# bnbowman/pbccs

Measured on AMD Instinct MI355X. Metric: CCS ZMWs/sec (and GCUPS) at 1/2/4/8 MI355X vs host-CPU ccs, higher is better.
Workload: dtype f64

## Files before the change

### pbccs_amd/csrc/engine.hip

```cpp
#include "engine.hpp"
#include "diploid_kernels.hpp"
#include "refine_repeats.hpp"

#include <hipcub/hipcub.hpp>

#include <algorithm>
#include <mutex>
#include <climits>
#include <cmath>
#include <cstdio>
#include <cstdlib>
#include <cstring>
#include <numeric>
#include <set>
#include <stdexcept>
#include <chrono>
#include <unordered_set>

namespace pbccs {

#define PBCCS_HIP(x)                                                         \
    do {                                                                     \
        hipError_t e_ = (x);                                                 \
        if (e_ != hipSuccess) throw DeviceError(hipGetErrorString(e_));      \
// ... 892 lines not shown
    b.prNot = 1.0 - kMismatchProbability;
    b.prThird = kMismatchProbability / 3.0;
    b.sdn = zmws_.empty() ? std::exp(12.5) : std::exp(zmws_[0].opt.scoreDiff);
    b.stats = profiling_ ? dStats_.ptr : nullptr;
    return b;
}

void ArrowBatch::FillReads(const std::vector<int>& readsIn)
{
    const StreamScope bound(stream_);
    constexpr int kPaths = 4;
    for (int r : readsIn) EnsureCapacity(r);
    auto promote = [&](int r, int p) {
        HRead& h = reads_[r];
        int q = p + 1;
        if (q == 2 && (long long)h.seq.size() + 1 > 4LL * kCoopTallRows) q = 3;
        h.fillPath = q;
        if (q >= 2 && q < kPaths) {
            const long long I = (long long)h.seq.size(), J = h.te - h.ts;
            const bool ck = ckptAll_ > 0 || (ckptK_ > 0 && J >= ckptMinLen_);
            const long long K = ck ? std::max(ckptAll_, ckptK_) : 1;
            const long long want = (I + 1) * (J + 1) / kTallFirstDiv / K + (ck ? 2 * (kCkptTail + 1) * (I + 1) : 0) + 64;
            if (want > h.valCap) {
                h.valCap = want;
                h.valA = valTop_;
                h.valB = valTop_ + h.valCap;
                valTop_ += 2 * h.valCap;
                descDirty_ = true;
            }
        }
        return q;
    };
    Relayout(readsIn);
    std::vector<int> todo[kPaths], serial, done;
    for (int r : readsIn) {
        const int p = reads_[r].fillPath;
        if (p >= kPaths) serial.push_back(r);
        else todo[p].push_back(r);
    }
    auto words = [&](int r) {
        return (int)(reads_[r].seq.size() + 7) / 8 + (reads_[r].te - reads_[r].ts + 8) / 8;
    };
    constexpr int tallG = 64;
    static const int tallRows = env_int("PBCCS_TALL_ROWS", kTallRowsPerLane) == 1 ? 1 : 2;
    const long long chunk = (long long)tallG * tallRows;
    const long long tallGroupLds = (long long)kCoopLdsBytes;
    auto full_rows = [&](int maxI) { return ((long long)maxI + chunk) / chunk * chunk; };
    constexpr int narrowG = kNarrowGroupLanes;
    constexpr int narrowRows = 1;
    auto rows_for = [&](int p, int maxI, int w) -> int {
        if (p == 0) return 0;
        if (p == 1)
            return (64 / narrowG) * coop_group_bytes(kCoopNarrowRows, w, 0) <= kCoopLdsBytes
                       ? kCoopNarrowRows : 0;
        const long long room = (tallGroupLds - (long long)coop_group_bytes(0, w, 0)) / 16 / 64 * 64;
        const long long full = full_rows(maxI);
        if (p == 2) {
            const long long want = std::min<long long>(kCoopTallRows, full);
            return room >= want ? (int)want : 0;
        }
        static const long long hybLds = (long long)env_int("PBCCS_HYBRID_LDS_KB", (int)(kCoopLdsBytes >> 10)) << 10;
        static const long long hybRows = env_int("PBCCS_HYBRID_ROWS", kHybridRows);
        const long long hroom = (std::min<long long>(hybLds, 160 << 10) - (long long)coop_group_bytes(0, w, 0)) / 16 / 64 * 64;
        const long long want = std::min(std::min(full, hroom), hybRows);
        return want >= 64 ? (int)want : 0;
    };
    static const bool pathTrace = std::getenv("PBCCS_FILL_PATHS") != nullptr;
    static const bool pathTrace2 = pathTrace && std::getenv("PBCCS_FILL_PATHS")[0] == '2';
    static const bool fillWork = std::getenv("PBCCS_FILL_WORK") != nullptr;
    for (int attempt = 0;; ++attempt) {
        for (int p = 0; p < kPaths; ++p) {
            std::vector<int> keep;
            for (int r : todo[p]) {
                if (rows_for(p, (int)reads_[r].seq.size(), words(r)) > 0) keep.push_back(r);
                else if (p + 1 < kPaths) todo[p + 1].push_back(r);
                else {
                    reads_[r].fillPath = kPaths;
                    serial.push_back(r);
                }
            }
            todo[p].swap(keep);
        }
        if (std::all_of(todo, todo + kPaths, [](const std::vector<int>& v) { return v.empty(); })) break;
        if (attempt > 8) throw DeviceError("band storage keeps overflowing");
        auto quick = [&](int x) { return reads_[x].filled && reads_[x].flips == 0 ? 1 : 0; };
        auto high = [&](int x) {
            const HRead& h = reads_[x];
            return h.filled && std::max(h.usedA, h.usedB) > 16LL * (h.te - h.ts + 1) ? 0 : 1;
        };
        for (int p = 0; p < kPaths; ++p) {
            auto& v = todo[p];
            if (p >= 2) {
                std::stable_sort(v.begin(), v.end(), [&](int x, int y) {
                    return std::max(reads_[x].usedA, reads_[x].usedB) > std::max(reads_[y].usedA, reads_[y].usedB);
                });
// ... 1517 lines not shown
```

### pbccs_amd/csrc/fill_coop.hip

```cpp
#include "arrow_device.hpp"
#include "arrow_kernels.hpp"
#include "coop_chain.hpp"

#include <algorithm>
#include <cstdlib>
#include <stdexcept>

namespace pbccs {
namespace {

using namespace coop;

template <int G>
struct Task {
    Group<G> g;
    int I, J, L, start;
    const unsigned* rdW;
    const unsigned* tpW;
    const double* ctx;
    double* lds0;
    double* lds1;
    double* glob0;
    double* glob1;
    int hcap;
    int rowsCap;
    bool gcol;
    int ckK;
    bool chainExit;
    int slackDiv;
    double prNot, prThird, sdn;
    double sdnInvLow;
    double sdnInvHigh;
    double devScale;
    double sdnInv;
    int r;
    double* pool;
    unsigned long long* bump;
    long long limit;
    long long* gA;
    long long* gB;
    long long* gCap;

    bool split;
    __device__ __forceinline__ int lrow(int k) const { return split ? (k & 1) * (hcap >> 1) + (k >> 1) : k; }
    __device__ __forceinline__ double* cptr(int b, int k) const
    {
        if (!gcol) return lds0 + (b ? hcap : 0) + lrow(k);
        return k < hcap ? lds0 + (b ? hcap : 0) + lrow(k) : glob0 + (b ? glob1 - glob0 : 0) + (k - hcap);
    }
    __device__ __forceinline__ double cget(int b, int k) const { return *cptr(b, k); }
    __device__ __forceinline__ void cset(int b, int k, double v) const { *cptr(b, k) = v; }
    __device__ __forceinline__ int TBase(int idx) const
    {
        return nib(tpW, max(idx, 0));
    }
    __device__ __forceinline__ int TCtx(int idx) const
    {
        return (start + idx + 1 < L) ? ctx_code(TBase(idx), TBase(idx + 1)) : kCtxZero;
    }
    __device__ __forceinline__ int RB(int x) const
    {
        return nib(rdW, x);
    }
};

struct PassOut {
    long long used;
    long long stored;
    double last;
    double sumL;
    bool tall;
    bool changed;
    bool regrow;
    int maxH;
    double dev;
    int unc;
};

struct Work {
    bool on;
    long long steps;
    long long issues;
};
__device__ __forceinline__ void count_issue(Work& W)
{
    if (W.on) {
        const unsigned long long act = __ballot(1);
        if ((int)(threadIdx.x & 63) == __ffsll((long long)act) - 1) W.issues += 1;
    }
}

__device__ __forceinline__ void col_fence(bool gcol)
{
    if (gcol) __builtin_amdgcn_fence(__ATOMIC_ACQ_REL, "workgroup");
}

__device__ __forceinline__ bool thr_ge(double x, double pm, double lo, double hi, bool& amb)
{
    const bool ge = x >= pm * hi;
    const bool lt = x < pm * lo;
    amb = pm != 0.0 && (pm < 0x1p-960 || (!ge && !lt));
    return ge || pm == 0.0;
}

__device__ __forceinline__ double scan_col_dev(double D, int chunks, int rowsPerChunk)
{
    return D + (4.0 * (double)chunks * (double)rowsPerChunk + 40.0 * (double)chunks + 8.0) * kUnitRoundoff;
}
__device__ __forceinline__ bool near_thr(double x, double t, double margin)
{
    const double mx = fmax(x, t);
    return mx > 0.0 && fabs(x - t) <= margin * mx;
}

template <int G>
__device__ __forceinline__ void copy_vals(int lane, double* __restrict__ dst, const double* __restrict__ src, long long n)
{
    long long k = lane;
    for (; k + 3 * G < n; k += 4 * G) {
        const double x0 = src[k], x1 = src[k + G], x2 = src[k + 2 * G], x3 = src[k + 3 * G];
        dst[k] = x0;
        dst[k + G] = x1;
        dst[k + 2 * G] = x2;
        dst[k + 3 * G] = x3;
    }
    for (; k < n; k += G) dst[k] = src[k];
}

template <int G>
__device__ bool regrow_bands(const Task<G>& T, Band& m, Band& o, bool mIsAlpha, long long need, long long keepO)
{
    if (!T.bump) return false;
    const long long full = (long long)(T.I + 1) * (T.J + 1) + 1;
    long long cap = max(need, keepO);
    cap = max(min(cap + cap / T.slackDiv + 64, full), max(need, keepO));
    unsigned long long base = 0;
    if (T.g.lane == 0) base = atomicAdd(T.bump, (unsigned long long)(2 * cap));
    base = (unsigned long long)__shfl((long long)base, 0, G);
    if (base + 2 * (unsigned long long)cap > (unsigned long long)T.limit) return false;
    __threadfence();
    double* na = T.pool + base;
    double* nb = na + cap;
    double* nm = mIsAlpha ? na : nb;
    double* no = mIsAlpha ? nb : na;
    copy_vals<G>(T.g.lane, no, o.val, keepO);
// ... 21 lines not shown
#pragma unroll
            for (int q = 0; q < 8; ++q) v[q] = m.L(k + q);
#pragma unroll
            for (int q = 0; q < 8; ++q) s = s + v[q];
        }
        for (; k <= J; ++k) s = s + m.L(k);
    }
    return T.g.bcast(s, 0);
}

#ifndef PBCCS_TALL_PREFETCH
#define PBCCS_TALL_PREFETCH 1
#endif
template <int G, int R, bool SCAN, bool GC>
__device__ PassOut coop_alpha(const Task<G>& T, Band& a, Band& o, bool guided, bool selfValid, bool& ovf, long long keepO,
                              Work& W)
{
    constexpr int CH = G * R;
    constexpr bool PF = GC || (G == 64 && PBCCS_TALL_PREFETCH && !SCAN);
    constexpr bool PFS = GC || (G == 64 && PBCCS_TALL_PREFETCH);
    const Band* guide = guided ? &o : nullptr;
    const int I = T.I, J = T.J, lane = T.g.lane;
    PassOut out{0, 0, 0.0, 0.0, false, !selfValid, false, 1, 0.0, 0};
    bool counting = false;
    (void)keepO;
    if (a.cap < 1) ovf = true;
    if (lane == 0) {
        if (!ovf) a.V(0) = 1.0;
        a.R(0) = make_int2(0, 1);
        a.O(0) = 0;
        a.L(0) = 0.0;
    }
    int prev = 0, cur = 1;
    if (lane == 0) T.cset(prev, 0, 1.0);
    int pb = 0, pe = 1;
    double D = 0.0;
    int unc = 0;
    long long used = 1, stored = 1;
    int hb = 1, he = 1;
    int prevCtx = kCtxZero;
    int curBase = T.TBase(0), curCtx = T.TCtx(0);
    int tA = T.TBase(1), tB = T.TBase(2);
    double myF = 1.0;
    int2 gR = make_int2(0, 0), sR = make_int2(0, 0), gN = make_int2(0, 0), sN = make_int2(0, 0);
    {
        const int jj = G == 64 ? 1 + lane : 1;
        if (guide && jj < J) gN = guide->R(jj);
        if (selfValid && jj < J) sN = a.R(jj);
    }
    for (int j = 1; j < J; ++j) {
        const int jb = (j - 1) & (G - 1);
        int gx = 0, gy = 0, sx = 0, sy = 0;
        if constexpr (G == 64) {
            if (jb == 0) {
                gR = gN;
                sR = sN;
                const int jj = j + G + lane;
                if (guide && jj < J) gN = guide->R(jj);
                if (selfValid && jj < J) sN = a.R(jj);
            }
            if (guide) { gx = T.g.bcast(gR.x, jb); gy = T.g.bcast(gR.y, jb); }
            if (selfValid) { sx = T.g.bcast(sR.x, jb); sy = T.g.bcast(sR.y, jb); }
        } else {
            gR = gN;
            sR = sN;
            if (guide && j + 1 < J) gN = guide->R(j + 1);
            if (selfValid && j + 1 < J) sN = a.R(j + 1);
            gx = gR.x; gy = gR.y; sx = sR.x; sy = sR.y;
        }
        (void)jb;
        if (guide) {
            if (gx < gy) { hb = min(gx, hb); he = max(gy, he); }
        }
        if (selfValid) {
            if (sx < sy) { hb = min(sx, hb); he = max(sy, he); }
        }
        const int reqEnd = min(I, he);
        const int nextBase = tA, nextCtx = (T.start + j + 1 < T.L) ? ctx_code(tA, tB) : kCtxZero;
        const int tC = T.TBase(j + 2);
        const double* cp = T.ctx + curCtx * kCtxStride;
        const double* pp = T.ctx + prevCtx * kCtxStride;
        const double pMatch = pp[kM], pDel = pp[kD];
        const double cBranch = cp[kB], cStick3 = cp[kS3];
        const int b = hb;
        double mx = 0.0, aLast[R];
        int e = b, nc = 0;
        if (b < I) {
            double carry = 0.0;
            auto load_prev = [&](int ibx, double (&dst)[R + 1]) {
#pragma unroll
                for (int q = 0; q <= R; ++q) {
                    const int row = ibx - 1 + q;
                    dst[q] = (row >= pb && row < pe) ? T.cget(prev, row - pb) : 0.0;
                }
            };
            double pvN[R + 1];
            if constexpr (PF) load_prev(b + lane * R, pvN);
            for (int i0 = b;; i0 += CH) {
                if ((nc + 1) * CH > T.rowsCap) {
                    out.tall = true;
                    out.used = used;
                    W.steps += nc;
                    return out;
                }
                count_issue(W);
                const int ib = i0 + lane * R;
                double m[R], k[R], d[R], x[R];
                {
                    double pv[R + 1];
                    if constexpr (PF) {
#pragma unroll
                        for (int q = 0; q <= R; ++q) pv[q] = pvN[q];
                        load_prev(ib + CH, pvN);
                    } else {
                        load_prev(ib, pv);
                    }
#pragma unroll
                    for (int r = 0; r < R; ++r) {
                        const int i = ib + r;
                        const int rb = (i >= 1 && i <= I) ? T.RB(i - 1) : 15;
                        const double mpe = pv[r] * (rb == curBase ? T.prNot : T.prThird);
                        m[r] = (i == 1 && j == 1) ? mpe : ((i != 1 && j != 1) ? mpe * pMatch : 0.0);
                        k[r] = (i > 1) ? (rb == nextBase ? cBranch : cStick3) : 0.0;
                        d[r] = (j > 1) ? pv[r + 1] * pDel : 0.0;
                        x[r] = 0.0;
                    }
                }
                bool nz = false;
#pragma unroll
                for (int r = 0; r < R; ++r) nz = nz || m[r] != 0.0 || d[r] != 0.0;
                const unsigned long long nzb = T.g.bits(nz);
                if (carry != 0.0 || nzb != 0) {
                    const int startLane = ((G == 64 || R > 1) && carry == 0.0) ? __ffsll((long long)nzb) - 1 : 0;
                    if constexpr (R == 1) {
                        const int i = ib;
                        if (G == 64 && T.chainExit) {
                            auto maybe_stop = [&](double xv) {
                                const double pmv = fmax(mx, prefix_max<G>(xv));
                                return T.g.bits((i + 1 >= I) || (xv < pmv * T.sdnInvLow && i + 1 >= reqEnd));
                            };
                            x[0] = insertion_chain64_exit(m[0], k[0], d[0], carry, min(reqEnd, I) - 1 - i0, maybe_stop,
                                                          startLane);
                        } else {
                            x[0] = insertion_chain<G>(m[0], k[0], d[0], carry);
                        }
                    } else {
                        auto maybe_stop = [&](const double (&xv)[R]) {
                            double lp = xv[0];
#pragma unroll
                            for (int r = 1; r < R; ++r) lp = fmax(lp, xv[r]);
                            const double ex = shift_up<G>(prefix_max<G>(lp), 0.0);
                            double run = fmax(mx, ex);
                            bool st = false;
#pragma unroll
                            for (int r = 0; r < R; ++r) {
                                run = fmax(run, xv[r]);
                                const int i = ib + r;
                                st = st || (i + 1 >= I) || (xv[r] < run * T.sdnInvLow && i + 1 >= reqEnd);
                            }
                            return T.g.bits(st);
                        };
                        const int firstRow = min(reqEnd, I) - 1 - i0;
                        if constexpr (SCAN) {
                            scan_chain64<R>(m, k, d, carry, x);
                        } else {
                            insertion_chain_rows<G, R>(m, k, d, carry, x, firstRow < 0 ? 0 : firstRow / R, T.chainExit,
                                                       startLane, maybe_stop);
                        }
                    }
                }
                double pmR[R];
                if constexpr (R == 1) {
                    pmR[0] = fmax(mx, prefix_max<G>(x[0]));
                } else {
                    double lp = x[0];
#pragma unroll
                    for (int r = 1; r < R; ++r) lp = fmax(lp, x[r]);
                    double run = fmax(mx, shift_up<G>(prefix_max<G>(lp), 0.0));
#pragma unroll
                    for (int r = 0; r < R; ++r) {
                        run = fmax(run, x[r]);
                        pmR[r] = run;
                    }
                }
                bool ge[R], amb = false;
#pragma unroll
                for (int r = 0; r < R; ++r) {
                    const int i = ib + r;
                    bool a;
                    ge[r] = thr_ge(x[r], pmR[r], T.sdnInvLow, T.sdnInvHigh, a);
                    amb = amb || (a && i + 1 < I && i + 1 >= reqEnd);
                }
                if (__ballot(amb) != 0) {
#pragma unroll
                    for (int r = 0; r < R; ++r) ge[r] = x[r] >= pmR[r] / T.sdn;
                }
                int fs = R;
#pragma unroll
                for (int r = R - 1; r >= 0; --r) {
                    const int i = ib + r;
                    const bool cont = (i + 1 < I) && (ge[r] || i + 1 < reqEnd);
                    if (!cont) fs = r;
                }
                const unsigned long long stop = T.g.bits(fs < R);
                const int lastLane = stop ? (__ffsll((long long)stop) - 1) : (G - 1);
                double pmAt = pmR[R - 1];
#pragma unroll
                for (int r = 0; r < R - 1; ++r)
                    if (r == fs) pmAt = pmR[r];
                if (SCAN && i0 + CH >= reqEnd) {
                    const double mg = T.devScale * (2.0 * scan_col_dev(D, nc + 1, CH) + 8.0 * kUnitRoundoff);
                    const int rsStop = stop ? T.g.bcast(fs, lastLane) : R;
                    bool u = false;
#pragma unroll
                    for (int r = 0; r < R; ++r) {
                        const int i = ib + r;
                        const bool matters = (i + 1 < I) && (i + 1 >= reqEnd);
                        const bool upto = !stop || lane < lastLane || (lane == lastLane && r <= rsStop);
                        u = u || (matters && upto && near_thr(x[r], pmR[r] * T.sdnInv, mg));
                    }
                    if (T.g.bits(u) != 0) unc |= 1;
                }
                mx = T.g.bcast(pmAt, lastLane);
                ++nc;
                if (stop) {
                    const int rs = R == 1 ? 0 : T.g.bcast(fs, lastLane);
                    e = i0 + lastLane * R + rs + 1;
#pragma unroll
                    for (int r = 0; r < R; ++r) aLast[r] = x[r];
                    break;
                }
#pragma unroll
                for (int r = 0; r < R; ++r) T.cset(cur, (nc - 1) * CH + lane * R + r, x[r]);
                carry = T.g.bcast_last(x[R - 1]);
            }
        }
        const bool keep = T.ckK == 0 || ckpt_col_a(j, J, T.ckK);
        const long long add = keep ? e - b : 0;
        if (!ovf && !counting && stored + add + 1 > a.cap) {
            if (T.bump) counting = true;
            else ovf = true;
        }
        const bool store = !ovf && !counting && keep;
        const double thrF = mx / T.sdn;
        const bool scale = (mx != 0.0 && mx != 1.0);
        int nhb = e;
        bool found = false;
        const double mh = SCAN ? T.devScale * (3.0 * scan_col_dev(D, nc, CH) + 4.0 * kUnitRoundoff) : 0.0;
        auto load_cur = [&](int cx, double (&dst)[R]) {
#pragma unroll
            for (int r = 0; r < R; ++r) dst[r] = (cx == nc - 1) ? aLast[r] : T.cget(cur, cx * CH + lane * R + r);
        };
        double xN[R];
        if constexpr (PFS) load_cur(0, xN);
#pragma unroll 2
        for (int c = 0; c < nc; ++c) {
            int fh = R;
            double vv[R];
            double xc[R];
            if constexpr (PFS) {
#pragma unroll
                for (int r = 0; r < R; ++r) xc[r] = xN[r];
                if (c + 1 < nc) load_cur(c + 1, xN);
            } else {
                load_cur(c, xc);
            }
#pragma unroll
            for (int r = 0; r < R; ++r) {
                const int kk = c * CH + lane * R + r;
                const bool ok = b + kk < e;
                const double x = xc[r];
                const double v = scale ? x / mx : x;
                if (ok) {
                    T.cset(cur, kk, v);
                    if (store && stored + kk < a.cap) a.V(stored + kk) = v;
                }
                if (fh == R && ok && !(v < thrF)) fh = r;
                vv[r] = ok ? v : -1.0;
            }
            const unsigned long long hit = T.g.bits(fh < R);
            if constexpr (SCAN) {
                if (!found) {
                    const int hl = hit ? __ffsll((long long)hit) - 1 : G;
                    const int fhl = hit ? T.g.bcast(fh, hl) : R;
                    bool u = false;
#pragma unroll
                    for (int r = 0; r < R; ++r)
                        u = u || (vv[r] >= 0.0 && (lane < hl || (lane == hl && r <= fhl)) && near_thr(vv[r], thrF, mh));
                    if (T.g.bits(u) != 0) unc |= 2;
                }
            }
            if (!found && hit) {
                const int hl = __ffsll((long long)hit) - 1;
                nhb = b + c * CH + hl * R + (R == 1 ? 0 : T.g.bcast(fh, hl));
                found = true;
            }
        }
        if constexpr (SCAN) D = scan_col_dev(D, nc, CH) + kUnitRoundoff;
        if (!counting && stored + add > a.cap) ovf = true;
        out.changed = out.changed || b != sx || e != sy;
        out.maxH = max(out.maxH, e - b);
        if (lane == 0 && !counting) {
            a.R(j) = make_int2(b, e);
            a.O(j) = (int)stored;
        }
        if (lane == jb) myF = scale ? mx : 1.0;
        if ((jb == G - 1 || j == J - 1) && !counting && lane <= jb) a.L(j - jb + lane) = (myF != 1.0) ? log(myF) : 0.0;
        used += e - b;
        stored += add;
        W.steps += nc;
        col_fence(T.gcol && nc * CH > T.hcap);
        prev ^= 1;
        cur ^= 1;
        pb = b;
        pe = e;
        prevCtx = curCtx;
        curBase = nextBase;
        curCtx = nextCtx;
        tA = tB;
        tB = tC;
        he = e;
        hb = nhb;
    }
    const double em = (T.RB(I - 1) == T.TBase(J - 1)) ? T.prNot : T.prThird;
    const bool lastIn = I - 1 >= pb && I - 1 < pe;
    const double lik = (lastIn ? T.cget(prev, I - 1 - pb) : 0.0) * em;
    const double c = (0.0 < lik) ? lik : 0.0;
    double v = lik, ls = 0.0;
    if (c != 0.0 && c != 1.0) { v = lik / c; ls = log(c); }
    if (!ovf && !counting && stored + 1 > a.cap) {
        if (T.bump) counting = true;
        else ovf = true;
    }
    out.regrow = counting;
    if (lane == 0 && !counting) {
        if (!ovf) a.V(stored) = v;
        a.R(J) = make_int2(I, I + 1);
        a.O(J) = (int)stored;
        a.L(J) = ls;
    }
    out.used = used + 1;
    out.stored = stored + 1;
    out.last = v;
    if (!counting) out.sumL = finish_log_scales<G>(T, a, J);
    if constexpr (SCAN) {
        out.dev = T.devScale * (1.01 * (D + 4.0 * kUnitRoundoff) +
                                2.0 * (double)(J + 4) * kUnitRoundoff * (fabs(out.sumL) + fabs(log(fmax(v, 1e-300))) + 64.0));
        out.unc = unc | ((lastIn && v == 0.0) ? 1 : 0);
    }
    return out;
}

template <int G, int R, bool SCAN, bool GC>
__device__ PassOut coop_beta(const Task<G>& T, Band& bm, Band& o, bool guided, bool selfValid, bool& ovf, long long keepO,
                             Work& W)
{
    constexpr int CH = G * R;
    constexpr bool PF = GC || (G == 64 && PBCCS_TALL_PREFETCH && !SCAN);
    constexpr bool PFS = GC || (G == 64 && PBCCS_TALL_PREFETCH);
    const Band* guide = guided ? &o : nullptr;
    const int I = T.I, J = T.J, lane = T.g.lane;
    PassOut out{0, 0, 0.0, 0.0, false, !selfValid, false, 1, 0.0, 0};
    bool counting = false;
    (void)keepO;
    if (bm.cap < 1) ovf = true;
    if (lane == 0) {
        if (!ovf) bm.V(0) = 1.0;
        bm.R(J) = make_int2(I, I + 1);
        bm.O(J) = 0;
        bm.L(J) = 0.0;
    }
    int nxt = 0, cur = 1;
    if (lane == 0) T.cset(nxt, 0, 1.0);
    int pb = I, pe = I + 1;
    double D = 0.0;
    int unc = 0;
    long long used = 1, stored = 1;
    int hb = I, he = I;
    int nextBase = T.TBase(J - 1);
    int tA = T.TBase(J - 2), tB = nextBase;
    double myF = 1.0;
    int2 gR = make_int2(0, 0), sR = make_int2(0, 0), gN = make_int2(0, 0), sN = make_int2(0, 0);
    {
        const int jj = G == 64 ? J - 1 - lane : J - 1;
        if (guide && jj > 0) gN = guide->R(jj);
        if (selfValid && jj > 0) sN = bm.R(jj);
    }
    for (int j = J - 1; j > 0; --j) {
        const int jb = (J - 1 - j) & (G - 1);
        int gx = 0, gy = 0, sx = 0, sy = 0;
        if constexpr (G == 64) {
            if (jb == 0) {
                gR = gN;
                sR = sN;
                const int jj = j - G - lane;
                if (guide && jj > 0) gN = guide->R(jj);
                if (selfValid && jj > 0) sN = bm.R(jj);
            }
            if (guide) { gx = T.g.bcast(gR.x, jb); gy = T.g.bcast(gR.y, jb); }
            if (selfValid) { sx = T.g.bcast(sR.x, jb); sy = T.g.bcast(sR.y, jb); }
        } else {
            gR = gN;
            sR = sN;
            if (guide && j - 1 > 0) gN = guide->R(j - 1);
            if (selfValid && j - 1 > 0) sN = bm.R(j - 1);
            gx = gR.x; gy = gR.y; sx = sR.x; sy = sR.y;
        }
        (void)jb;
        const int curBase = tA, curCtx = (T.start + j < T.L) ? ctx_code(tA, tB) : kCtxZero;
        const int tC = T.TBase(j - 2);
        if (guide) {
            if (gx < gy) { hb = min(gx, hb); he = max(gy, he); }
        }
        if (selfValid) {
            if (sx < sy) { hb = min(sx, hb); he = max(sy, he); }
        }
        const int reqBegin = max(0, hb);
        const double* cp = T.ctx + curCtx * kCtxStride;
        const double cMatch = cp[kM], cDel = cp[kD], cBranch = cp[kB], cStick3 = cp[kS3];
        const int e = he;
        double mx = 0.0, aLast[R];
        int b = e, nc = 0;
        if (e - 1 > 0) {
            double carry = 0.0;
            auto load_next = [&](int obx, double (&dst)[R + 1]) {
#pragma unroll
                for (int q = 0; q <= R; ++q) {
                    const int row = e - obx - q;
                    dst[q] = (row >= pb && row < pe) ? T.cget(nxt, pe - 1 - row) : 0.0;
                }
            };
            double pvN[R + 1];
            if constexpr (PF) load_next(lane * R, pvN);
            for (int c = 0;; ++c) {
                if ((c + 1) * CH > T.rowsCap) {
                    out.tall = true;
                    out.used = used;
                    W.steps += nc;
                    return out;
                }
                count_issue(W);
                const int ob = c * CH + lane * R;
                double m[R], k[R], d[R], x[R];
                {
                    double pv[R + 1];
                    if constexpr (PF) {
#pragma unroll
                        for (int q = 0; q <= R; ++q) pv[q] = pvN[q];
                        load_next(ob + CH, pvN);
                    } else {
                        load_next(ob, pv);
                    }
#pragma unroll
                    for (int r = 0; r < R; ++r) {
                        const int i = e - 1 - ob - r;
                        const int nb = (i >= 0 && i < I) ? T.RB(i) : 15;
                        const bool same = nb == nextBase;
                        const double mpe = pv[r] * (same ? T.prNot : T.prThird);
                        m[r] = (i < I - 1) ? mpe * cMatch : ((i == I - 1 && j == J - 1) ? mpe : 0.0);
                        k[r] = (i < I - 1 && i > 0) ? (same ? cBranch : cStick3) : 0.0;
                        d[r] = (j < J - 1 && j > 0) ? pv[r + 1] * cDel : 0.0;
                        x[r] = 0.0;
                    }
                }
                bool nz = false;
#pragma unroll
                for (int r = 0; r < R; ++r) nz = nz || m[r] != 0.0 || d[r] != 0.0;
                const unsigned long long nzb = T.g.bits(nz);
                if (carry != 0.0 || nzb != 0) {
                    const int startLane = ((G == 64 || R > 1) && carry == 0.0) ? __ffsll((long long)nzb) - 1 : 0;
                    if constexpr (R == 1) {
                        const int i = e - 1 - ob;
                        if (G == 64 && T.chainExit) {
                            auto maybe_stop = [&](double xv) {
                                const double pmv = fmax(mx, prefix_max<G>(xv));
                                return T.g.bits((i - 1 <= 0) || (xv < pmv * T.sdnInvLow && i - 1 < reqBegin));
                            };
                            x[0] = insertion_chain64_exit(m[0], k[0], d[0], carry, e - 1 - max(1, reqBegin) - c * G,
                                                          maybe_stop, startLane);
                        } else {
                            x[0] = insertion_chain<G>(m[0], k[0], d[0], carry);
                        }
                    } else {
                        auto maybe_stop = [&](const double (&xv)[R]) {
                            double lp = xv[0];
#pragma unroll
                            for (int r = 1; r < R; ++r) lp = fmax(lp, xv[r]);
                            const double ex = shift_up<G>(prefix_max<G>(lp), 0.0);
                            double run = fmax(mx, ex);
                            bool st = false;
#pragma unroll
                            for (int r = 0; r < R; ++r) {
                                run = fmax(run, xv[r]);
                                const int i = e - 1 - ob - r;
                                st = st || (i - 1 <= 0) || (xv[r] < run * T.sdnInvLow && i - 1 < reqBegin);
                            }
                            return T.g.bits(st);
                        };
                        const int firstOff = e - 1 - max(1, reqBegin) - c * CH;
                        if constexpr (SCAN) {
                            scan_chain64<R>(m, k, d, carry, x);
                        } else {
                            insertion_chain_rows<G, R>(m, k, d, carry, x, firstOff < 0 ? 0 : firstOff / R, T.chainExit,
                                                       startLane, maybe_stop);
                        }
                    }
                }
                double pmR[R];
                if constexpr (R == 1) {
                    pmR[0] = fmax(mx, prefix_max<G>(x[0]));
                } else {
                    double lp = x[0];
#pragma unroll
                    for (int r = 1; r < R; ++r) lp = fmax(lp, x[r]);
                    double run = fmax(mx, shift_up<G>(prefix_max<G>(lp), 0.0));
#pragma unroll
                    for (int r = 0; r < R; ++r) {
                        run = fmax(run, x[r]);
                        pmR[r] = run;
                    }
                }
                bool ge[R], amb = false;
#pragma unroll
                for (int r = 0; r < R; ++r) {
                    const int i = e - 1 - ob - r;
                    bool a;
                    ge[r] = thr_ge(x[r], pmR[r], T.sdnInvLow, T.sdnInvHigh, a);
                    amb = amb || (a && i - 1 > 0 && i - 1 < reqBegin);
                }
                if (__ballot(amb) != 0) {
#pragma unroll
                    for (int r = 0; r < R; ++r) ge[r] = x[r] >= pmR[r] / T.sdn;
                }
                int fs = R;
#pragma unroll
                for (int r = R - 1; r >= 0; --r) {
                    const int i = e - 1 - ob - r;
                    const bool cont = (i - 1 > 0) && (ge[r] || i - 1 >= reqBegin);
                    if (!cont) fs = r;
                }
                const unsigned long long stop = T.g.bits(fs < R);
                const int lastLane = stop ? (__ffsll((long long)stop) - 1) : (G - 1);
                double pmAt = pmR[R - 1];
#pragma unroll
                for (int r = 0; r < R - 1; ++r)
                    if (r == fs) pmAt = pmR[r];
                if (SCAN && e - (c + 1) * CH - 1 < reqBegin) {
                    const double mg = T.devScale * (2.0 * scan_col_dev(D, nc + 1, CH) + 8.0 * kUnitRoundoff);
                    const int rsStop = stop ? T.g.bcast(fs, lastLane) : R;
                    bool u = false;
#pragma unroll
                    for (int r = 0; r < R; ++r) {
                        const int i = e - 1 - ob - r;
                        const bool matters = (i - 1 > 0) && (i - 1 < reqBegin);
                        const bool upto = !stop || lane < lastLane || (lane == lastLane && r <= rsStop);
                        u = u || (matters && upto && near_thr(x[r], pmR[r] * T.sdnInv, mg));
                    }
                    if (T.g.bits(u) != 0) unc |= 1;
                }
                mx = T.g.bcast(pmAt, lastLane);
                ++nc;
                if (stop) {
                    const int rs = R == 1 ? 0 : T.g.bcast(fs, lastLane);
                    b = e - 1 - (c * CH + lastLane * R + rs);
#pragma unroll
                    for (int r = 0; r < R; ++r) aLast[r] = x[r];
                    break;
                }
#pragma unroll
                for (int r = 0; r < R; ++r) T.cset(cur, ob + r, x[r]);
                carry = T.g.bcast_last(x[R - 1]);
            }
        }
        const bool keep = T.ckK == 0 || ckpt_col_b(j, J, T.ckK);
        const long long add = keep ? e - b : 0;
        if (!ovf && !counting && stored + add + 1 > bm.cap) {
            if (T.bump) counting = true;
            else ovf = true;
        }
        const bool store = !ovf && !counting && keep;
        const double thrF = mx / T.sdn;
        const bool scale = (mx != 0.0 && mx != 1.0);
        int nhe = b;
        bool found = false;
        const double mh = SCAN ? T.devScale * (3.0 * scan_col_dev(D, nc, CH) + 4.0 * kUnitRoundoff) : 0.0;
        auto load_cur = [&](int cx, double (&dst)[R]) {
#pragma unroll
            for (int r = 0; r < R; ++r) dst[r] = (cx == nc - 1) ? aLast[r] : T.cget(cur, cx * CH + lane * R + r);
        };
        double xN[R];
        if constexpr (PFS) load_cur(0, xN);
#pragma unroll 2
        for (int c = 0; c < nc; ++c) {
            int fh = R;
            double vv[R];
            double xc[R];
            if constexpr (PFS) {
#pragma unroll
                for (int r = 0; r < R; ++r) xc[r] = xN[r];
                if (c + 1 < nc) load_cur(c + 1, xN);
            } else {
                load_cur(c, xc);
            }
#pragma unroll
            for (int r = 0; r < R; ++r) {
                const int off = c * CH + lane * R + r;
                const bool ok = e - 1 - off >= b;
                const double x = xc[r];
                const double v = scale ? x / mx : x;
                if (ok) {
                    T.cset(cur, off, v);
                    if (store && stored + off < bm.cap) bm.V(stored + off) = v;
                }
                if (fh == R && ok && !(v < thrF)) fh = r;
                vv[r] = ok ? v : -1.0;
            }
            const unsigned long long hit = T.g.bits(fh < R);
            if constexpr (SCAN) {
                if (!found) {
                    const int hl = hit ? __ffsll((long long)hit) - 1 : G;
                    const int fhl = hit ? T.g.bcast(fh, hl) : R;
                    bool u = false;
#pragma unroll
                    for (int r = 0; r < R; ++r)
                        u = u || (vv[r] >= 0.0 && (lane < hl || (lane == hl && r <= fhl)) && near_thr(vv[r], thrF, mh));
                    if (T.g.bits(u) != 0) unc |= 2;
                }
            }
            if (!found && hit) {
                const int hl = __ffsll((long long)hit) - 1;
                nhe = e - (c * CH + hl * R + (R == 1 ? 0 : T.g.bcast(fh, hl)));
                found = true;
            }
        }
        if constexpr (SCAN) D = scan_col_dev(D, nc, CH) + kUnitRoundoff;
        if (!counting && stored + add > bm.cap) ovf = true;
        out.changed = out.changed || b != sx || e != sy;
        out.maxH = max(out.maxH, e - b);
        if (lane == 0 && !counting) {
            bm.R(j) = make_int2(b, e);
            bm.O(j) = (int)stored;
        }
        if (lane == jb) myF = scale ? mx : 1.0;
        if ((jb == G - 1 || j == 1) && !counting && lane <= jb) bm.L(j + jb - lane) = (myF != 1.0) ? log(myF) : 0.0;
        used += e - b;
        stored += add;
        W.steps += nc;
        col_fence(T.gcol && nc * CH > T.hcap);
        nxt ^= 1;
        cur ^= 1;
        pb = b;
        pe = e;
        hb = b;
        he = nhe;
        nextBase = curBase;
        tB = tA;
        tA = tC;
    }
    const double em = (T.TBase(0) == T.RB(0)) ? T.prNot : T.prThird;
    const bool lastIn = 1 >= pb && 1 < pe;
    const double raw = em * (lastIn ? T.cget(nxt, pe - 2) : 0.0);
    const double c = (0.0 < raw) ? raw : 0.0;
    double v = raw, ls = 0.0;
    if (c != 0.0 && c != 1.0) { v = raw / c; ls = log(c); }
    if (!ovf && !counting && stored + 1 > bm.cap) {
        if (T.bump) counting = true;
        else ovf = true;
    }
    out.regrow = counting;
    if (lane == 0 && !counting) {
        if (!ovf) bm.V(stored) = v;
        bm.R(0) = make_int2(0, 1);
        bm.O(0) = (int)stored;
        bm.L(0) = ls;
    }
    out.used = used + 1;
    out.stored = stored + 1;
    out.last = v;
    if (!counting) out.sumL = finish_log_scales<G>(T, bm, J);
    if constexpr (SCAN) {
        out.dev = T.devScale * (1.01 * (D + 4.0 * kUnitRoundoff) +
                                2.0 * (double)(J + 4) * kUnitRoundoff * (fabs(out.sumL) + fabs(log(fmax(v, 1e-300))) + 64.0));
        out.unc = unc | ((lastIn && v == 0.0) ? 1 : 0);
    }
    return out;
}

}

template <int G, bool GC, int R, bool SCAN>
__device__ __forceinline__ void fill_read(const DevBatch& B, const CoopFill& F, const int* __restrict__ reads, int n,
                                          int t, unsigned char* gbase)
{
    const int lane = threadIdx.x & (G - 1);
// ... 22 lines not shown
            for (int k = lane; k < kCtxDoubles; k += G) ctx[k] = zc[k];
        }
        if (!bad) {
            const char* rd = B.seqPool + B.rSeqOff[r];
            for (int w = lane; w < (I + 7) / 8; w += G) {
                unsigned word = 0;
                for (int q = 0; q < 8; ++q) {
                    const int x = 8 * w + q;
                    word |= (unsigned)(x < I ? base_code(rd[x]) : kBaseOther) << (4 * q);
                }
                rdW[w] = word;
            }
            for (int w = lane; w < (J + 8) / 8; w += G) {
                unsigned word = 0;
                for (int q = 0; q < 8; ++q) {
                    const int x = 8 * w + q;
                    const int g = tv.start + x;
                    word |= (unsigned)((x <= J && g < tv.L) ? base_code(tv.T[g]) : kBaseOther) << (4 * q);
                }
                tpW[w] = word;
            }
        }
    }
    __builtin_amdgcn_fence(__ATOMIC_ACQ_REL, "workgroup");
    if (!valid) return;
    if (bad) {
        if (lane == 0) B.rStatus[r] = (I < 1 || J < 1) ? kFillBadInput : kFillOverflow;
        return;
    }

    Task<G> T;
    T.g.lane = lane;
    T.g.base = (int)threadIdx.x & ~(G - 1);
    T.I = I;
    T.J = J;
    T.L = tv.L;
    T.start = tv.start;
    T.rdW = rdW;
    T.tpW = tpW;
    T.ctx = ctx;
    T.lds0 = col;
    T.lds1 = col + F.hcap;
    T.glob0 = GC ? F.colScratch + (size_t)t * 2 * F.gRows : nullptr;
    T.glob1 = GC ? T.glob0 + F.gRows : nullptr;
    T.hcap = F.hcap;
    T.split = R == 2;
    T.rowsCap = GC ? F.hcap + F.gRows : F.hcap;
    T.gcol = GC;
    T.chainExit = F.chainExit;
    T.ckK = B.rCkpt ? B.rCkpt[r] : 0;
    T.slackDiv = max(1, F.regrowSlackDiv);
    T.prNot = B.prNot;
    T.prThird = B.prThird;
    T.sdn = B.sdn;
    T.sdnInvLow = (1.0 / B.sdn) * (1.0 - F.thrMargin);
    T.sdnInvHigh = (1.0 / B.sdn) * (1.0 + F.thrMargin);
    T.devScale = F.devScale;
    T.sdnInv = 1.0 / B.sdn;
    T.r = r;
    T.pool = B.valPool;
    T.bump = F.valBump;
    T.limit = F.valLimit;
    T.gA = F.rValA;
    T.gB = F.rValB;
    T.gCap = F.rValCap;

    const long long cb = B.rColBase[r];
    Band a, bm;
    a.range = B.aRange + cb;
    a.off = B.aOff + cb;
    a.ls = B.aLs + cb;
    a.val = B.valPool + B.rValA[r];
    a.cap = B.rValCap[r];
    bm.range = B.bRange + cb;
    bm.off = B.bOff + cb;
    bm.ls = B.bLs + cb;
    bm.val = B.valPool + B.rValB[r];
    bm.cap = B.rValCap[r];

// ... 200 lines not shown
```

Before: 3306.

## Specialize coop fill LDS addressing and skip band threshold tests off the tail

Makes the split-plane row layout a compile-time template parameter and adds direct LDS pointer/selection helpers for the non-global-column wide-group path. Scalarizes wavefront-uniform values with readfirstlane, loads several read bases from one packed 64-bit word, and folds branchy emission/deletion factors into multiplications. It also skips the per-chunk threshold/ambiguity ballot unless the chunk reaches the required band end, and uses non-short-circuit boolean ops to reduce divergence. It adds an env knob for the first fill path and makes some env lookups non-static, which adds a small per-call host cost.

Result: faster. 3603, median of 6 (+9.0%).

```diff
diff --git a/pbccs_amd/csrc/engine.hip b/pbccs_amd/csrc/engine.hip
--- a/pbccs_amd/csrc/engine.hip
+++ b/pbccs_amd/csrc/engine.hip
@@ -948,8 +948,10 @@
         return q;
     };
     Relayout(readsIn);
+    const int firstPath = std::min(std::max(env_int("PBCCS_FILL_FIRST_PATH", 1), 1), 3);
     std::vector<int> todo[kPaths], serial, done;
     for (int r : readsIn) {
+        if (reads_[r].fillPath < firstPath) reads_[r].fillPath = firstPath;
         const int p = reads_[r].fillPath;
         if (p >= kPaths) serial.push_back(r);
         else todo[p].push_back(r);
@@ -958,7 +960,7 @@
         return (int)(reads_[r].seq.size() + 7) / 8 + (reads_[r].te - reads_[r].ts + 8) / 8;
     };
     constexpr int tallG = 64;
-    static const int tallRows = env_int("PBCCS_TALL_ROWS", kTallRowsPerLane) == 1 ? 1 : 2;
+    const int tallRows = env_int("PBCCS_TALL_ROWS", kTallRowsPerLane) == 1 ? 1 : 2;
     const long long chunk = (long long)tallG * tallRows;
     const long long tallGroupLds = (long long)kCoopLdsBytes;
     auto full_rows = [&](int maxI) { return ((long long)maxI + chunk) / chunk * chunk; };
@@ -975,8 +977,8 @@
             const long long want = std::min<long long>(kCoopTallRows, full);
             return room >= want ? (int)want : 0;
         }
-        static const long long hybLds = (long long)env_int("PBCCS_HYBRID_LDS_KB", (int)(kCoopLdsBytes >> 10)) << 10;
-        static const long long hybRows = env_int("PBCCS_HYBRID_ROWS", kHybridRows);
+        const long long hybLds = (long long)env_int("PBCCS_HYBRID_LDS_KB", (int)(kCoopLdsBytes >> 10)) << 10;
+        const long long hybRows = env_int("PBCCS_HYBRID_ROWS", kHybridRows);
         const long long hroom = (std::min<long long>(hybLds, 160 << 10) - (long long)coop_group_bytes(0, w, 0)) / 16 / 64 * 64;
         const long long want = std::min(std::min(full, hroom), hybRows);
         return want >= 64 ? (int)want : 0;
diff --git a/pbccs_amd/csrc/fill_coop.hip b/pbccs_amd/csrc/fill_coop.hip
--- a/pbccs_amd/csrc/fill_coop.hip
+++ b/pbccs_amd/csrc/fill_coop.hip
@@ -41,15 +41,49 @@
     long long* gB;
     long long* gCap;
 
-    bool split;
-    __device__ __forceinline__ int lrow(int k) const { return split ? (k & 1) * (hcap >> 1) + (k >> 1) : k; }
+    __device__ __forceinline__ int uni(int x) const
+    {
+        if constexpr (G == 64) return __builtin_amdgcn_readfirstlane(x);
+        return x;
+    }
+
+    template <int R>
+    __device__ __forceinline__ int lrow(int k) const
+    {
+        static_assert(R <= 2, "the split layout has two planes");
+        return R > 1 ? (k & 1) * (hcap >> 1) + (k >> 1) : k;
+    }
+    template <int R>
     __device__ __forceinline__ double* cptr(int b, int k) const
     {
-        if (!gcol) return lds0 + (b ? hcap : 0) + lrow(k);
-        return k < hcap ? lds0 + (b ? hcap : 0) + lrow(k) : glob0 + (b ? glob1 - glob0 : 0) + (k - hcap);
-    }
-    __device__ __forceinline__ double cget(int b, int k) const { return *cptr(b, k); }
-    __device__ __forceinline__ void cset(int b, int k, double v) const { *cptr(b, k) = v; }
+        if (!gcol) return lds0 + (b ? hcap : 0) + lrow<R>(k);
+        return k < hcap ? lds0 + (b ? hcap : 0) + lrow<R>(k) : glob0 + (b ? glob1 - glob0 : 0) + (k - hcap);
+    }
+    template <int R>
+    __device__ __forceinline__ double cget(int b, int k) const { return *cptr<R>(b, k); }
+    template <int R>
+    __device__ __forceinline__ void cset(int b, int k, double v) const { *cptr<R>(b, k) = v; }
+    template <int R>
+    __device__ __forceinline__ double* lptr(int b, int c, int r) const
+    {
+        static_assert(R <= 2, "the split layout has two planes");
+        return lds0 + (b ? hcap : 0) + (R > 1 ? r * (hcap >> 1) : 0) + c * G + g.lane;
+    }
+    template <int R>
+    __device__ __forceinline__ double lget_sel(int b, int s, int h) const
+    {
+        static_assert(R <= 2, "the split layout has two planes");
+        const bool in = (unsigned)(s + R * g.lane) < (unsigned)h;
+        double v;
+        if constexpr (R > 1) {
+            const int half = hcap >> 1;
+            const int p = min(max((s >> 1) + g.lane, 0), half - 1);
+            v = lds0[(b ? hcap : 0) + (s & 1) * half + p];
+        } else {
+            v = lds0[(b ? hcap : 0) + min(max(s + g.lane, 0), hcap - 1)];
+        }
+        return in ? v : 0.0;
+    }
     __device__ __forceinline__ int TBase(int idx) const
     {
         return nib(tpW, max(idx, 0));
@@ -61,6 +95,25 @@
     __device__ __forceinline__ int RB(int x) const
     {
         return nib(rdW, x);
+    }
+    template <int R>
+    __device__ __forceinline__ void RBs(int x0, int (&rb)[R]) const
+    {
+        static_assert(R <= 9, "R codes from a clamped position span at most two words");
+        const int xc = min(max(x0, 0), I - 1);
+        if constexpr (R == 1) {
+            const int v = nib(rdW, xc);
+            rb[0] = (unsigned)x0 < (unsigned)I ? v : 15;
+        } else {
+            const int w = xc >> 3;
+            const unsigned long long bits = (unsigned long long)rdW[w] | ((unsigned long long)rdW[w + 1] << 32);
+#pragma unroll
+            for (int r = 0; r < R; ++r) {
+                const int x = x0 + r;
+                const int v = (int)(bits >> (((x - 8 * w) & 15) << 2)) & 15;
+                rb[r] = (unsigned)x < (unsigned)I ? v : 15;
+            }
+        }
     }
 };
 
@@ -99,18 +152,18 @@
 {
     const bool ge = x >= pm * hi;
     const bool lt = x < pm * lo;
-    amb = pm != 0.0 && (pm < 0x1p-960 || (!ge && !lt));
-    return ge || pm == 0.0;
+    amb = (pm != 0.0) & ((pm < 0x1p-960) | (!ge & !lt));
+    return ge | (pm == 0.0);
 }
 
 __device__ __forceinline__ double scan_col_dev(double D, int chunks, int rowsPerChunk)
 {
-    return D + (4.0 * (double)chunks * (double)rowsPerChunk + 40.0 * (double)chunks + 8.0) * kUnitRoundoff;
+    return D + (double)(4 * chunks * rowsPerChunk + 40 * chunks + 8) * kUnitRoundoff;
 }
 __device__ __forceinline__ bool near_thr(double x, double t, double margin)
 {
     const double mx = fmax(x, t);
-    return mx > 0.0 && fabs(x - t) <= margin * mx;
+    return (mx > 0.0) & (fabs(x - t) <= margin * mx);
 }
 
 template <int G>
@@ -198,7 +251,7 @@
         a.L(0) = 0.0;
     }
     int prev = 0, cur = 1;
-    if (lane == 0) T.cset(prev, 0, 1.0);
+    if (lane == 0) T.template cset<R>(prev, 0, 1.0);
     int pb = 0, pe = 1;
     double D = 0.0;
     int unc = 0;
@@ -241,27 +294,34 @@
         if (selfValid) {
             if (sx < sy) { hb = min(sx, hb); he = max(sy, he); }
         }
-        const int reqEnd = min(I, he);
+        const int reqEnd = T.uni(min(I, he));
         const int nextBase = tA, nextCtx = (T.start + j + 1 < T.L) ? ctx_code(tA, tB) : kCtxZero;
         const int tC = T.TBase(j + 2);
         const double* cp = T.ctx + curCtx * kCtxStride;
         const double* pp = T.ctx + prevCtx * kCtxStride;
         const double pMatch = pp[kM], pDel = pp[kD];
         const double cBranch = cp[kB], cStick3 = cp[kS3];
-        const int b = hb;
+        const double mFac = (j == 1) ? 1.0 : pMatch, dFac = (j > 1) ? pDel : 0.0;
+        const int b = T.uni(hb);
         double mx = 0.0, aLast[R];
         int e = b, nc = 0;
         if (b < I) {
             double carry = 0.0;
-            auto load_prev = [&](int ibx, double (&dst)[R + 1]) {
+            const int hPrev = T.uni(pe - pb);
+            auto load_prev = [&](int i0x, double (&dst)[R + 1]) {
+                const int s0 = T.uni(i0x - 1 - pb);
 #pragma unroll
                 for (int q = 0; q <= R; ++q) {
-                    const int row = ibx - 1 + q;
-                    dst[q] = (row >= pb && row < pe) ? T.cget(prev, row - pb) : 0.0;
+                    if constexpr (GC || G < 64) {
+                        const int row = i0x + lane * R - 1 + q;
+                        dst[q] = (row >= pb && row < pe) ? T.template cget<R>(prev, row - pb) : 0.0;
+                    } else {
+                        dst[q] = T.template lget_sel<R>(prev, s0 + q, hPrev);
+                    }
                 }
             };
             double pvN[R + 1];
-            if constexpr (PF) load_prev(b + lane * R, pvN);
+            if constexpr (PF) load_prev(b, pvN);
             for (int i0 = b;; i0 += CH) {
                 if ((nc + 1) * CH > T.rowsCap) {
                     out.tall = true;
@@ -277,18 +337,20 @@
                     if constexpr (PF) {
 #pragma unroll
                         for (int q = 0; q <= R; ++q) pv[q] = pvN[q];
-                        load_prev(ib + CH, pvN);
+                        load_prev(i0 + CH, pvN);
                     } else {
-                        load_prev(ib, pv);
-                    }
+                        load_prev(i0, pv);
+                    }
+                    int rbs[R];
+                    T.template RBs<R>(ib - 1, rbs);
 #pragma unroll
                     for (int r = 0; r < R; ++r) {
                         const int i = ib + r;
-                        const int rb = (i >= 1 && i <= I) ? T.RB(i - 1) : 15;
+                        const int rb = rbs[r];
                         const double mpe = pv[r] * (rb == curBase ? T.prNot : T.prThird);
-                        m[r] = (i == 1 && j == 1) ? mpe : ((i != 1 && j != 1) ? mpe * pMatch : 0.0);
+                        m[r] = mpe * (((i == 1) == (j == 1)) ? mFac : 0.0);
                         k[r] = (i > 1) ? (rb == nextBase ? cBranch : cStick3) : 0.0;
-                        d[r] = (j > 1) ? pv[r + 1] * pDel : 0.0;
+                        d[r] = pv[r + 1] * dFac;
                         x[r] = 0.0;
                     }
                 }
@@ -349,26 +411,30 @@
                         pmR[r] = run;
                     }
                 }
-                bool ge[R], amb = false;
-#pragma unroll
-                for (int r = 0; r < R; ++r) {
-                    const int i = ib + r;
-                    bool a;
-                    ge[r] = thr_ge(x[r], pmR[r], T.sdnInvLow, T.sdnInvHigh, a);
-                    amb = amb || (a && i + 1 < I && i + 1 >= reqEnd);
-                }
-                if (__ballot(amb) != 0) {
-#pragma unroll
-                    for (int r = 0; r < R; ++r) ge[r] = x[r] >= pmR[r] / T.sdn;
-                }
+                const bool tests = G < 64 || i0 + CH >= reqEnd;
                 int fs = R;
-#pragma unroll
-                for (int r = R - 1; r >= 0; --r) {
-                    const int i = ib + r;
-                    const bool cont = (i + 1 < I) && (ge[r] || i + 1 < reqEnd);
-                    if (!cont) fs = r;
-                }
-                const unsigned long long stop = T.g.bits(fs < R);
+                unsigned long long stop = 0;
+                if (tests) {
+                    bool ge[R], amb = false;
+#pragma unroll
+                    for (int r = 0; r < R; ++r) {
+                        const int i = ib + r;
+                        bool a;
+                        ge[r] = thr_ge(x[r], pmR[r], T.sdnInvLow, T.sdnInvHigh, a);
+                        amb = amb || (a && i + 1 < I && i + 1 >= reqEnd);
+                    }
+                    if (__ballot(amb) != 0) {
+#pragma unroll
+                        for (int r = 0; r < R; ++r) ge[r] = x[r] >= pmR[r] / T.sdn;
+                    }
+#pragma unroll
+                    for (int r = R - 1; r >= 0; --r) {
+                        const int i = ib + r;
+                        const bool cont = (i + 1 < I) && (ge[r] || i + 1 < reqEnd);
+                        if (!cont) fs = r;
+                    }
+                    stop = T.g.bits(fs < R);
+                }
                 const int lastLane = stop ? (__ffsll((long long)stop) - 1) : (G - 1);
                 double pmAt = pmR[R - 1];
 #pragma unroll
@@ -383,7 +449,7 @@
                         const int i = ib + r;
                         const bool matters = (i + 1 < I) && (i + 1 >= reqEnd);
                         const bool upto = !stop || lane < lastLane || (lane == lastLane && r <= rsStop);
-                        u = u || (matters && upto && near_thr(x[r], pmR[r] * T.sdnInv, mg));
+                        u = u | (matters & upto & near_thr(x[r], pmR[r] * T.sdnInv, mg));
                     }
                     if (T.g.bits(u) != 0) unc |= 1;
                 }
@@ -397,7 +463,10 @@
                     break;
                 }
 #pragma unroll
-                for (int r = 0; r < R; ++r) T.cset(cur, (nc - 1) * CH + lane * R + r, x[r]);
+                for (int r = 0; r < R; ++r) {
+                    if constexpr (GC) T.template cset<R>(cur, (nc - 1) * CH + lane * R + r, x[r]);
+                    else *T.template lptr<R>(cur, nc - 1, r) = x[r];
+                }
                 carry = T.g.bcast_last(x[R - 1]);
             }
         }
@@ -412,10 +481,19 @@
         const bool scale = (mx != 0.0 && mx != 1.0);
         int nhb = e;
         bool found = false;
-        const double mh = SCAN ? T.devScale * (3.0 * scan_col_dev(D, nc, CH) + 4.0 * kUnitRoundoff) : 0.0;
+        const double Dc = SCAN ? scan_col_dev(D, nc, CH) : 0.0;
+        const double mh = SCAN ? T.devScale * (3.0 * Dc + 4.0 * kUnitRoundoff) : 0.0;
+        const int capRows = (int)max(0LL, min((long long)0x7fffffff, a.cap - stored));
         auto load_cur = [&](int cx, double (&dst)[R]) {
 #pragma unroll
-            for (int r = 0; r < R; ++r) dst[r] = (cx == nc - 1) ? aLast[r] : T.cget(cur, cx * CH + lane * R + r);
+            for (int r = 0; r < R; ++r) {
+                if constexpr (GC) {
+                    dst[r] = (cx == nc - 1) ? aLast[r] : T.template cget<R>(cur, cx * CH + lane * R + r);
+                } else {
+                    const double ld = *T.template lptr<R>(cur, cx, r);
+                    dst[r] = (cx == nc - 1) ? aLast[r] : ld;
+                }
+            }
         };
         double xN[R];
         if constexpr (PFS) load_cur(0, xN);
@@ -438,8 +516,9 @@
                 const double x = xc[r];
                 const double v = scale ? x / mx : x;
                 if (ok) {
-                    T.cset(cur, kk, v);
-                    if (store && stored + kk < a.cap) a.V(stored + kk) = v;
+                    if constexpr (GC) T.template cset<R>(cur, kk, v);
+                    else *T.template lptr<R>(cur, c, r) = v;
+                    if (store && kk < capRows) a.V(stored + kk) = v;
                 }
                 if (fh == R && ok && !(v < thrF)) fh = r;
                 vv[r] = ok ? v : -1.0;
@@ -452,7 +531,7 @@
                     bool u = false;
 #pragma unroll
                     for (int r = 0; r < R; ++r)
-                        u = u || (vv[r] >= 0.0 && (lane < hl || (lane == hl && r <= fhl)) && near_thr(vv[r], thrF, mh));
+                        u = u | ((vv[r] >= 0.0) & ((lane < hl) | ((lane == hl) & (r <= fhl))) & near_thr(vv[r], thrF, mh));
                     if (T.g.bits(u) != 0) unc |= 2;
                 }
             }
@@ -462,7 +541,7 @@
                 found = true;
             }
         }
-        if constexpr (SCAN) D = scan_col_dev(D, nc, CH) + kUnitRoundoff;
+        if constexpr (SCAN) D = Dc + kUnitRoundoff;
         if (!counting && stored + add > a.cap) ovf = true;
         out.changed = out.changed || b != sx || e != sy;
         out.maxH = max(out.maxH, e - b);
@@ -490,7 +569,7 @@
     }
     const double em = (T.RB(I - 1) == T.TBase(J - 1)) ? T.prNot : T.prThird;
     const bool lastIn = I - 1 >= pb && I - 1 < pe;
-    const double lik = (lastIn ? T.cget(prev, I - 1 - pb) : 0.0) * em;
+    const double lik = (lastIn ? T.template cget<R>(prev, I - 1 - pb) : 0.0) * em;
     const double c = (0.0 < lik) ? lik : 0.0;
     double v = lik, ls = 0.0;
     if (c != 0.0 && c != 1.0) { v = lik / c; ls = log(c); }
@@ -537,7 +616,7 @@
         bm.L(J) = 0.0;
     }
     int nxt = 0, cur = 1;
-    if (lane == 0) T.cset(nxt, 0, 1.0);
+    if (lane == 0) T.template cset<R>(nxt, 0, 1.0);
     int pb = I, pe = I + 1;
     double D = 0.0;
     int unc = 0;
@@ -581,23 +660,30 @@
         if (selfValid) {
             if (sx < sy) { hb = min(sx, hb); he = max(sy, he); }
         }
-        const int reqBegin = max(0, hb);
+        const int reqBegin = T.uni(max(0, hb));
         const double* cp = T.ctx + curCtx * kCtxStride;
         const double cMatch = cp[kM], cDel = cp[kD], cBranch = cp[kB], cStick3 = cp[kS3];
-        const int e = he;
+        const int e = T.uni(he);
+        const double dFac = (j < J - 1 && j > 0) ? cDel : 0.0, mLast = (j == J - 1) ? 1.0 : 0.0;
         double mx = 0.0, aLast[R];
         int b = e, nc = 0;
         if (e - 1 > 0) {
             double carry = 0.0;
-            auto load_next = [&](int obx, double (&dst)[R + 1]) {
+            const int hNext = T.uni(pe - pb);
+            auto load_next = [&](int o0x, double (&dst)[R + 1]) {
+                const int s0 = T.uni(pe - 1 - e + o0x);
 #pragma unroll
                 for (int q = 0; q <= R; ++q) {
-                    const int row = e - obx - q;
-                    dst[q] = (row >= pb && row < pe) ? T.cget(nxt, pe - 1 - row) : 0.0;
+                    if constexpr (GC || G < 64) {
+                        const int row = e - (o0x + lane * R) - q;
+                        dst[q] = (row >= pb && row < pe) ? T.template cget<R>(nxt, pe - 1 - row) : 0.0;
+                    } else {
+                        dst[q] = T.template lget_sel<R>(nxt, s0 + q, hNext);
+                    }
                 }
             };
             double pvN[R + 1];
-            if constexpr (PF) load_next(lane * R, pvN);
+            if constexpr (PF) load_next(0, pvN);
             for (int c = 0;; ++c) {
                 if ((c + 1) * CH > T.rowsCap) {
                     out.tall = true;
@@ -613,19 +699,21 @@
                     if constexpr (PF) {
 #pragma unroll
                         for (int q = 0; q <= R; ++q) pv[q] = pvN[q];
-                        load_next(ob + CH, pvN);
+                        load_next((c + 1) * CH, pvN);
                     } else {
-                        load_next(ob, pv);
-                    }
+                        load_next(c * CH, pv);
+                    }
+                    int rbs[R];
+                    T.template RBs<R>(e - ob - R, rbs);
 #pragma unroll
                     for (int r = 0; r < R; ++r) {
                         const int i = e - 1 - ob - r;
-                        const int nb = (i >= 0 && i < I) ? T.RB(i) : 15;
+                        const int nb = rbs[R - 1 - r];
                         const bool same = nb == nextBase;
                         const double mpe = pv[r] * (same ? T.prNot : T.prThird);
-                        m[r] = (i < I - 1) ? mpe * cMatch : ((i == I - 1 && j == J - 1) ? mpe : 0.0);
+                        m[r] = mpe * (i < I - 1 ? cMatch : (i == I - 1 ? mLast : 0.0));
                         k[r] = (i < I - 1 && i > 0) ? (same ? cBranch : cStick3) : 0.0;
-                        d[r] = (j < J - 1 && j > 0) ? pv[r + 1] * cDel : 0.0;
+                        d[r] = pv[r + 1] * dFac;
                         x[r] = 0.0;
                     }
                 }
@@ -686,26 +774,30 @@
                         pmR[r] = run;
                     }
                 }
-                bool ge[R], amb = false;
-#pragma unroll
-                for (int r = 0; r < R; ++r) {
-                    const int i = e - 1 - ob - r;
-                    bool a;
-                    ge[r] = thr_ge(x[r], pmR[r], T.sdnInvLow, T.sdnInvHigh, a);
-                    amb = amb || (a && i - 1 > 0 && i - 1 < reqBegin);
-                }
-                if (__ballot(amb) != 0) {
-#pragma unroll
-                    for (int r = 0; r < R; ++r) ge[r] = x[r] >= pmR[r] / T.sdn;
-                }
+                const bool tests = G < 64 || e - (c + 1) * CH - 1 < max(reqBegin, 1);
                 int fs = R;
-#pragma unroll
-                for (int r = R - 1; r >= 0; --r) {
-                    const int i = e - 1 - ob - r;
-                    const bool cont = (i - 1 > 0) && (ge[r] || i - 1 >= reqBegin);
-                    if (!cont) fs = r;
-                }
-                const unsigned long long stop = T.g.bits(fs < R);
+                unsigned long long stop = 0;
+                if (tests) {
+                    bool ge[R], amb = false;
+#pragma unroll
+                    for (int r = 0; r < R; ++r) {
+                        const int i = e - 1 - ob - r;
+                        bool a;
+                        ge[r] = thr_ge(x[r], pmR[r], T.sdnInvLow, T.sdnInvHigh, a);
+                        amb = amb || (a && i - 1 > 0 && i - 1 < reqBegin);
+                    }
+                    if (__ballot(amb) != 0) {
+#pragma unroll
+                        for (int r = 0; r < R; ++r) ge[r] = x[r] >= pmR[r] / T.sdn;
+                    }
+#pragma unroll
+                    for (int r = R - 1; r >= 0; --r) {
+                        const int i = e - 1 - ob - r;
+                        const bool cont = (i - 1 > 0) && (ge[r] || i - 1 >= reqBegin);
+                        if (!cont) fs = r;
+                    }
+                    stop = T.g.bits(fs < R);
+                }
                 const int lastLane = stop ? (__ffsll((long long)stop) - 1) : (G - 1);
                 double pmAt = pmR[R - 1];
 #pragma unroll
@@ -720,7 +812,7 @@
                         const int i = e - 1 - ob - r;
                         const bool matters = (i - 1 > 0) && (i - 1 < reqBegin);
                         const bool upto = !stop || lane < lastLane || (lane == lastLane && r <= rsStop);
-                        u = u || (matters && upto && near_thr(x[r], pmR[r] * T.sdnInv, mg));
+                        u = u | (matters & upto & near_thr(x[r], pmR[r] * T.sdnInv, mg));
                     }
                     if (T.g.bits(u) != 0) unc |= 1;
                 }
@@ -734,7 +826,10 @@
                     break;
                 }
 #pragma unroll
-                for (int r = 0; r < R; ++r) T.cset(cur, ob + r, x[r]);
+                for (int r = 0; r < R; ++r) {
+                    if constexpr (GC) T.template cset<R>(cur, ob + r, x[r]);
+                    else *T.template lptr<R>(cur, c, r) = x[r];
+                }
                 carry = T.g.bcast_last(x[R - 1]);
             }
         }
@@ -749,10 +844,19 @@
         const bool scale = (mx != 0.0 && mx != 1.0);
         int nhe = b;
         bool found = false;
-        const double mh = SCAN ? T.devScale * (3.0 * scan_col_dev(D, nc, CH) + 4.0 * kUnitRoundoff) : 0.0;
+        const double Dc = SCAN ? scan_col_dev(D, nc, CH) : 0.0;
+        const double mh = SCAN ? T.devScale * (3.0 * Dc + 4.0 * kUnitRoundoff) : 0.0;
+        const int capRows = (int)max(0LL, min((long long)0x7fffffff, bm.cap - stored));
         auto load_cur = [&](int cx, double (&dst)[R]) {
 #pragma unroll
-            for (int r = 0; r < R; ++r) dst[r] = (cx == nc - 1) ? aLast[r] : T.cget(cur, cx * CH + lane * R + r);
+            for (int r = 0; r < R; ++r) {
+                if constexpr (GC) {
+                    dst[r] = (cx == nc - 1) ? aLast[r] : T.template cget<R>(cur, cx * CH + lane * R + r);
+                } else {
+                    const double ld = *T.template lptr<R>(cur, cx, r);
+                    dst[r] = (cx == nc - 1) ? aLast[r] : ld;
+                }
+            }
         };
         double xN[R];
         if constexpr (PFS) load_cur(0, xN);
@@ -775,8 +879,9 @@
                 const double x = xc[r];
                 const double v = scale ? x / mx : x;
                 if (ok) {
-                    T.cset(cur, off, v);
-                    if (store && stored + off < bm.cap) bm.V(stored + off) = v;
+                    if constexpr (GC) T.template cset<R>(cur, off, v);
+                    else *T.template lptr<R>(cur, c, r) = v;
+                    if (store && off < capRows) bm.V(stored + off) = v;
                 }
                 if (fh == R && ok && !(v < thrF)) fh = r;
                 vv[r] = ok ? v : -1.0;
@@ -789,7 +894,7 @@
                     bool u = false;
 #pragma unroll
                     for (int r = 0; r < R; ++r)
-                        u = u || (vv[r] >= 0.0 && (lane < hl || (lane == hl && r <= fhl)) && near_thr(vv[r], thrF, mh));
+                        u = u | ((vv[r] >= 0.0) & ((lane < hl) | ((lane == hl) & (r <= fhl))) & near_thr(vv[r], thrF, mh));
                     if (T.g.bits(u) != 0) unc |= 2;
                 }
             }
@@ -799,7 +904,7 @@
                 found = true;
             }
         }
-        if constexpr (SCAN) D = scan_col_dev(D, nc, CH) + kUnitRoundoff;
+        if constexpr (SCAN) D = Dc + kUnitRoundoff;
         if (!counting && stored + add > bm.cap) ovf = true;
         out.changed = out.changed || b != sx || e != sy;
         out.maxH = max(out.maxH, e - b);
@@ -825,7 +930,7 @@
     }
     const double em = (T.TBase(0) == T.RB(0)) ? T.prNot : T.prThird;
     const bool lastIn = 1 >= pb && 1 < pe;
-    const double raw = em * (lastIn ? T.cget(nxt, pe - 2) : 0.0);
+    const double raw = em * (lastIn ? T.template cget<R>(nxt, pe - 2) : 0.0);
     const double c = (0.0 < raw) ? raw : 0.0;
     double v = raw, ls = 0.0;
     if (c != 0.0 && c != 1.0) { v = raw / c; ls = log(c); }
@@ -914,8 +1019,8 @@
     Task<G> T;
     T.g.lane = lane;
     T.g.base = (int)threadIdx.x & ~(G - 1);
-    T.I = I;
-    T.J = J;
+    T.I = T.uni(I);
+    T.J = T.uni(J);
     T.L = tv.L;
     T.start = tv.start;
     T.rdW = rdW;
@@ -926,7 +1031,6 @@
     T.glob0 = GC ? F.colScratch + (size_t)t * 2 * F.gRows : nullptr;
     T.glob1 = GC ? T.glob0 + F.gRows : nullptr;
     T.hcap = F.hcap;
-    T.split = R == 2;
     T.rowsCap = GC ? F.hcap + F.gRows : F.hcap;
     T.gcol = GC;
     T.chainExit = F.chainExit;
```
